# weidafeng/Efficient-SlowFast

Hardware: AMD Instinct MI355X
Metric: clips/sec (8x8 224^2 SlowFast-R50+CMDA, train step fwd+bwd+allreduce+SGD) (higher is better)
Workload: dtype f32

## Files before the change

### efficient-slowfast_amd/sfhip/__init__.py

```python
import ctypes
import os

import torch

_HERE = os.path.dirname(os.path.abspath(__file__))
_LIB_PATH = os.environ.get("SF_LIB") or os.path.join(_HERE, "libsfhip.so")
_lib = None

ACT_NONE, ACT_RELU, ACT_SIGMOID, ACT_SOFTMAX, ACT_HSIGMOID, ACT_RELU6 = 0, 1, 2, 3, 4, 5


def _act(relu):
    return ACT_RELU6 if relu == 6 else (ACT_RELU if relu else ACT_NONE)
SF_EINVAL, SF_EALIGN, SF_ELAUNCH, SF_ENOTTAKEN = -1, -2, -3, -4
_ERR = {-1: "SF_EINVAL (inconsistent descriptor)", -2: "SF_EALIGN", -3: "SF_ELAUNCH (hip launch failed)",
        -4: "SF_ENOTTAKEN (shape not served by this specialised entry point)"}


class SfhipError(RuntimeError):
    pass


class ConvDesc(ctypes.Structure):
    _fields_ = [(n, ctypes.c_int) for n in (
        "N", "Ti", "Hi", "Wi", "Cin", "in_cs", "in_coff", "To", "Ho", "Wo", "Cout", "out_cs", "out_coff",
        "out_cmul", "kT", "kH", "kW", "sT", "sH", "sW", "pT", "pH", "pW", "dT", "dH", "dW", "cin_pad", "act",
        "res_cs", "res_coff", "transposed", "os_T", "os_H", "os_W", "oo_T", "oo_H", "oo_W", "ob_T", "ob_H", "ob_W")]


class PoolDesc(ctypes.Structure):
    _fields_ = [(n, ctypes.c_int) for n in (
        "N", "Ti", "Hi", "Wi", "C", "in_cs", "in_coff", "To", "Ho", "Wo", "out_cs", "out_coff",
        "kT", "kH", "kW", "sT", "sH", "sW", "pT", "pH", "pW", "is_avg")]


EXPORTS = [
    "sf_abi_version", "sf_build_arch", "sf_ncthw_to_ndhwc", "sf_ndhwc_to_ncthw", "sf_conv_fwd", "sf_dwconv_fwd",
    "sf_pool_fwd", "sf_maxpool_fwd_arg", "sf_maxpool_bwd_arg", "sf_tmax_mean_ws_floats", "sf_tmax_mean", "sf_gate_apply", "sf_attn_fwd", "sf_head_act_mean",
    "sf_copy_channels", "sf_channel_stats_ws_floats", "sf_channel_stats", "sf_affine_fwd", "sf_bn_train_stats",
    "sf_conv_wgrad_splits", "sf_conv_wgrad", "sf_bn_bwd_ws_floats", "sf_bn_bwd_reduce", "sf_bn_bwd_apply",
    "sf_attn_bwd", "sf_maxpool_bwd", "sf_tmax_dot", "sf_eca_bwd_apply", "sf_eca_gate_bwd", "sf_bcast_add", "sf_rowdot", "sf_axpy", "sf_act_bwd",
    "sf_dwconv_dgrad", "sf_dwconv_wgrad_ws_floats", "sf_dwconv_wgrad", "sf_gather_add",
    "sf_bn_train_stats_split", "sf_affine_fwd_split", "sf_bn_bwd_reduce_split", "sf_bn_bwd_apply_split",
    "sf_clip_prologue", "sf_conv_wgrad_finish", "sf_bn_bwd_reduce_acc", "sf_row_softmax_fwd", "sf_row_softmax_bwd",
    "sf_attn_bwd_fused_ws_floats", "sf_attn_bwd_fused", "sf_pack_conv_weight", "sf_conv_fwd_ws_floats",
    "sf_conv_fwd_ws", "sf_attn_fwd_ws_floats", "sf_attn_fwd_ws", "sf_affine_fwd_mask", "sf_bn_bwd_apply_first", "sf_maxpool_bwd_first",
    "sf_conv_tune", "sf_conv_stats_ws_floats", "sf_conv_fwd_stats", "sf_bn_train_stats_merge",
    "sf_attn_products_per_fp32", "sf_pack_conv_weights", "sf_attn_bwd_variant", "sf_attn_tune",
    "sf_bx_planes_elems", "sf_bx_split", "sf_bx_split_batched", "sf_conv_rows_parts", "sf_conv_pw_ws_floats", "sf_conv_pw_stats_floats", "sf_conv_fwd_pw", "sf_conv_bx_ws_floats", "sf_conv_fwd_bx", "sf_conv_wgrad_bx_splits",
    "sf_conv_wgrad_bx_ws_floats", "sf_conv_wgrad_bx",
    "sf_conv_fwd_grouped", "sf_conv_wgrad_grouped_splits", "sf_conv_wgrad_grouped", "sf_channel_shuffle",
    "sf_dwconv_wgrad_param", "sf_roi_tpool_fwd", "sf_roi_align_max_fwd", "sf_roi_align_max_bwd", "sf_sigmoid_bwd",
]
_LONG_RET = ("sf_tmax_mean_ws_floats", "sf_channel_stats_ws_floats", "sf_bn_bwd_ws_floats",
             "sf_dwconv_wgrad_ws_floats", "sf_attn_bwd_fused_ws_floats", "sf_conv_fwd_ws_floats",
             "sf_attn_fwd_ws_floats", "sf_conv_stats_ws_floats", "sf_bx_planes_elems", "sf_conv_bx_ws_floats",
             "sf_conv_wgrad_bx_ws_floats")


def lib_path():
    return _LIB_PATH


def lib():
    global _lib
    if _lib is None:
        if not os.path.exists(_LIB_PATH):
            raise SfhipError(
                "libsfhip.so not found at %s — build it with `make -C efficient-slowfast_amd/csrc` "
                "(there is no CPU fallback for the SlowFast hot path)" % _LIB_PATH)
        L = ctypes.CDLL(_LIB_PATH)
        vp, ci, cl = ctypes.c_void_p, ctypes.c_int, ctypes.c_long
        L.sf_abi_version.restype = ci
        L.sf_build_arch.restype = ctypes.c_char_p
        L.sf_ncthw_to_ndhwc.argtypes = [vp, vp] + [ci] * 9 + [vp]
        L.sf_ndhwc_to_ncthw.argtypes = [vp, ci, ci, vp] + [ci] * 5 + [vp]
        L.sf_conv_fwd.argtypes = [ctypes.POINTER(ConvDesc)] + [vp] * 7
        L.sf_dwconv_fwd.argtypes = [ctypes.POINTER(ConvDesc)] + [vp] * 7
        L.sf_pool_fwd.argtypes = [ctypes.POINTER(PoolDesc), vp, vp, vp]
        L.sf_maxpool_fwd_arg.argtypes = [ctypes.POINTER(PoolDesc), vp, vp, vp, vp]
        L.sf_maxpool_bwd_arg.argtypes = [ctypes.POINTER(PoolDesc), vp, vp, ci, ci, vp, ci, ci, ci, vp]
        L.sf_tmax_mean_ws_floats.argtypes = [ci, ci]
        L.sf_tmax_mean_ws_floats.restype = cl
        L.sf_tmax_mean.argtypes = [vp, ci, ci] + [ci] * 6 + [vp, vp, vp]
        L.sf_gate_apply.argtypes = [vp, ci, ci] + [ci] * 6 + [vp, vp, vp, vp, ci, vp, ci, ci, vp]
# ... 54 lines not shown
        L.sf_conv_tune.argtypes = [ci, ci]
        L.sf_attn_tune.argtypes = [ci, ci]
        L.sf_bx_planes_elems.argtypes = [cl, ci]
        L.sf_bx_planes_elems.restype = cl
        L.sf_bx_split.argtypes = [vp, ci, ci, cl, ci, vp, vp]
        L.sf_bx_split_batched.argtypes = [vp, vp, ci, ci, vp]
        L.sf_conv_pw_ws_floats.argtypes = [ctypes.POINTER(ConvDesc), ci]
        L.sf_conv_pw_ws_floats.restype = cl
        L.sf_conv_rows_parts.argtypes = [ctypes.POINTER(ConvDesc)]
        L.sf_conv_pw_stats_floats.argtypes = [ctypes.POINTER(ConvDesc)]
        L.sf_conv_pw_stats_floats.restype = cl
        L.sf_conv_fwd_pw.argtypes = [ctypes.POINTER(ConvDesc)] + [vp] * 9 + [ctypes.POINTER(ctypes.c_int), vp]
        L.sf_conv_bx_ws_floats.argtypes = [ctypes.POINTER(ConvDesc), ci, ci]
        L.sf_conv_bx_ws_floats.restype = cl
        L.sf_conv_fwd_bx.argtypes = [ctypes.POINTER(ConvDesc)] + [vp] * 10
        L.sf_conv_wgrad_bx_splits.argtypes = [ctypes.POINTER(ConvDesc)]
        L.sf_conv_wgrad_bx_ws_floats.argtypes = [ctypes.POINTER(ConvDesc), ci, ci]
        L.sf_conv_wgrad_bx_ws_floats.restype = cl
        L.sf_conv_wgrad_bx.argtypes = [ctypes.POINTER(ConvDesc), vp, vp, vp, ci, ci, vp, vp, vp, vp]
        L.sf_attn_bwd_variant.argtypes = [ci, ci, ci]
        L.sf_row_softmax_fwd.argtypes = [vp, ci, ci, cl, ci, cf, vp]
        L.sf_row_softmax_bwd.argtypes = [vp, ci, ci, vp, ci, ci, cl, ci, cf, vp]
        L.sf_conv_wgrad_finish.argtypes = [vp, ci, ci, ci, ci, ci, ci, vp, ci, vp]
        L.sf_bn_bwd_reduce_acc.argtypes = [vp, ci, ci, vp, ci, ci, vp, ci, ci] + [ci] * 7 + [vp] * 5 + [vp, vp, vp]
        L.sf_bn_train_stats_split.argtypes = [vp, ci, ci, ci, cl, ci, ci, vp, vp, cf, cf] + [vp] * 9
        L.sf_affine_fwd_split.argtypes = [vp, ci, ci] + [ci] * 6 + [vp, vp, vp, ci, ci, ci, ci, vp, ci, ci, ci, vp]
        L.sf_bn_bwd_reduce_split.argtypes = [vp, ci, ci, vp, ci, ci, vp, ci, ci] + [ci] * 8 + [vp] * 5 + [vp]
        L.sf_bn_bwd_apply_split.argtypes = ([vp, ci, ci, vp, ci, ci, vp, ci, ci] + [ci] * 8 + [vp] * 5 +
                                            [vp, ci, ci, vp, ci, ci, vp])
        L.sf_roi_tpool_fwd.argtypes = [vp, ci, ci] + [ci] * 5 + [vp, vp]
        L.sf_roi_align_max_fwd.argtypes = [vp] + [ci] * 4 + [vp, ci, ci, cf, ci, vp, ci, ci, vp, vp]
        L.sf_roi_align_max_bwd.argtypes = [vp, ci, ci, vp, vp] + [ci] * 7 + [cf, ci, vp, ci, ci, ci, vp]
        L.sf_sigmoid_bwd.argtypes = [vp, vp, vp, cl, ci, vp]
        for name in EXPORTS:
            fn = getattr(L, name)
            if name != "sf_build_arch" and name not in _LONG_RET:
                fn.restype = ci
        _lib = L
    return _lib


def _check(rc, what):
    if rc != 0:
        raise SfhipError("%s failed: %s" % (what, _ERR.get(rc, rc)))


CALLS = 0


def _stream():
    global CALLS
    CALLS += 1
    return ctypes.c_void_p(torch.cuda.current_stream().cuda_stream)


def _ptr(t):
    return ctypes.c_void_p(t.data_ptr()) if t is not None else None


EVENT_TRACE = None


def _traced(tag, fn):
    if EVENT_TRACE is None:
        return fn()
    e0 = torch.cuda.Event(enable_timing=True)
# ... 600 lines not shown
    d = ConvDesc(x.N, x.T, x.H, x.W, cin, x.cs, x.coff, dz.T, dz.H, dz.W, cout, 0, 0, 1,
                 kT, kH, kW, stride[0], stride[1], stride[2], padding[0], padding[1], padding[2],
                 dilation[0], dilation[1], dilation[2], cin_pad, ACT_NONE, 0, 0, 0)
    nws = lib().sf_conv_wgrad_bx_ws_floats(ctypes.byref(d), 1 if x_planes is not None else 0,
                                           1 if dz_planes is not None else 0) if cin_pad == cin else 0
    if nws > 0:
        S = lib().sf_conv_wgrad_bx_splits(ctypes.byref(d))
        part = torch.empty((S, cout, kT * kH * kW, cin_pad), dtype=torch.float32, device=x.buf.device)
        ws = torch.empty((nws,), dtype=torch.float32, device=x.buf.device)
        rc = _traced(("conv", dz.rows, kT * kH * kW * cin, cout), lambda: lib().sf_conv_wgrad_bx(
            ctypes.byref(d), x.ptr(), _ptr(x_planes), dz.ptr(), dz.cs, dz.coff, _ptr(dz_planes), _ptr(part), _ptr(ws),
            _stream()))
        if rc in (SF_EALIGN, SF_ENOTTAKEN):
            nws = 0
        else:
            _check(rc, "sf_conv_wgrad_bx")
    if nws <= 0:
        S = lib().sf_conv_wgrad_splits(ctypes.byref(d))
        part = torch.empty((S, cout, kT * kH * kW, cin_pad), dtype=torch.float32, device=x.buf.device)
        _check(_traced(("conv", dz.rows, kT * kH * kW * cin, cout), lambda: lib().sf_conv_wgrad(
            ctypes.byref(d), x.ptr(), dz.ptr(), dz.cs, dz.coff, _ptr(part), _stream())), "sf_conv_wgrad")
    if finish_into is not None:
        dst, real_cin, fold_kw = finish_into
        assert dst.is_contiguous() and dst.dtype == torch.float32
        if S > 128 and cout * kT * kH * kW * cin_pad > 65536:
            part, S = part.sum(0, keepdim=True), 1
        assert dst.numel() == cout * real_cin * kT * kH * kW * max(fold_kw, 1), (dst.shape, cout, real_cin, kernel)
        _check(lib().sf_conv_wgrad_finish(_ptr(part), S, cout, kT * kH * kW, cin_pad, real_cin, fold_kw, _ptr(dst), 1,
                                          _stream()), "sf_conv_wgrad_finish")
        return None
    return part.sum(0) if S > 1 else part[0]


def conv_grouped(x, wp, groups, kernel, stride=(1, 1, 1), padding=(0, 0, 0), dilation=(1, 1, 1), scale=None,
                 bias=None, relu=False, res=None, out=None, shuffle=False, out_reserve=(0, 0)):
    _require_gpu(x.buf, "conv_grouped")
    cout, taps, cin_pad = wp.shape
    kT, kH, kW = kernel
    To = _out_dim(x.T, kT, stride[0], padding[0], dilation[0])
    Ho = _out_dim(x.H, kH, stride[1], padding[1], dilation[1])
    Wo = _out_dim(x.W, kW, stride[2], padding[2], dilation[2])
    if out is None:
        out = new_act(x, x.N, To, Ho, Wo, cout, out_reserve[0], out_reserve[1])
    assert (out.N, out.T, out.H, out.W, out.C) == (x.N, To, Ho, Wo, cout), (out, (x.N, To, Ho, Wo, cout))
    assert x.C % groups == 0 and cout % groups == 0 and cin_pad >= x.C // groups, (x, wp.shape, groups)
    d = ConvDesc(x.N, x.T, x.H, x.W, x.C, x.cs, x.coff, To, Ho, Wo, cout, out.cs, out.coff, 1,
                 kT, kH, kW, stride[0], stride[1], stride[2], padding[0], padding[1], padding[2],
                 dilation[0], dilation[1], dilation[2], cin_pad, _act(relu),
                 res.cs if res is not None else 0, res.coff if res is not None else 0, 0)
    if res is not None:
        assert res.rows == out.rows and res.C == cout
    tag = ("conv", d.N * d.To * d.Ho * d.Wo, taps * (x.C // groups), cout)
    _check(_traced(tag, lambda: lib().sf_conv_fwd_grouped(
        ctypes.byref(d), groups, 1 if shuffle else 0, x.ptr(), _ptr(wp), _ptr(scale), _ptr(bias),
        res.ptr() if res is not None else None, out.ptr(), _stream())), "sf_conv_fwd_grouped")
    return out


def conv_dgrad_grouped(dz, wtp, groups, x_like, kernel, stride=(1, 1, 1), padding=(0, 0, 0), dilation=(1, 1, 1),
                       out=None, accumulate=False):
    _require_gpu(dz.buf, "conv_dgrad_grouped")
    cin, taps, cout_pad = wtp.shape
    if out is None:
        out = new_act(dz, x_like.N, x_like.T, x_like.H, x_like.W, cin)
        accumulate = False
    assert (out.N, out.T, out.H, out.W, out.C) == (x_like.N, x_like.T, x_like.H, x_like.W, cin), (out, x_like)
# ... 10 lines not shown


def conv_wgrad_grouped(x, dz, groups, kernel, stride=(1, 1, 1), padding=(0, 0, 0), dilation=(1, 1, 1),
                       cin_pad=None, finish_into=None):
    _require_gpu(x.buf, "conv_wgrad_grouped")
    cin_g, cout = x.C // groups, dz.C
    assert x.C % groups == 0 and cout % groups == 0
    cin_pad = (cin_g + 15) // 16 * 16 if cin_pad is None else cin_pad
    kT, kH, kW = kernel
    d = ConvDesc(x.N, x.T, x.H, x.W, x.C, x.cs, x.coff, dz.T, dz.H, dz.W, cout, 0, 0, 1,
                 kT, kH, kW, stride[0], stride[1], stride[2], padding[0], padding[1], padding[2],
                 dilation[0], dilation[1], dilation[2], cin_pad, ACT_NONE, 0, 0, 0)
    S = lib().sf_conv_wgrad_grouped_splits(ctypes.byref(d), groups)
    if S <= 0:
        raise SfhipError("sf_conv_wgrad_grouped_splits: %d -> %d channels in %d groups" % (x.C, cout, groups))
    part = torch.empty((S, cout, kT * kH * kW, cin_pad), dtype=torch.float32, device=x.buf.device)
    _check(_traced(("conv", dz.rows, kT * kH * kW * cin_g, cout), lambda: lib().sf_conv_wgrad_grouped(
        ctypes.byref(d), groups, x.ptr(), dz.ptr(), dz.cs, dz.coff, _ptr(part), _stream())), "sf_conv_wgrad_grouped")
    if finish_into is not None:
        dst = finish_into
        assert dst.is_contiguous() and dst.dtype == torch.float32 and dst.numel() == cout * cin_g * kT * kH * kW
        _check(lib().sf_conv_wgrad_finish(_ptr(part), S, cout, kT * kH * kW, cin_pad, cin_g, 0, _ptr(dst), 1,
                                          _stream()), "sf_conv_wgrad_finish")
        return None
    return part.sum(0) if S > 1 else part[0]


def unpack_conv_weight_grad(dwp, shape):
    cout, cin, kT, kH, kW = shape
    return dwp[:, :, :cin].permute(0, 2, 1).reshape(cout, cin, kT, kH, kW).contiguous()


def bn_bwd(dy, y, z, mean, invstd, gamma, relu, rep=1, dres=None, dz_out=None, dgamma_out=None, nsplit=1,
           sync=None, grad_sink=None, mask=None, dres_overwrite=False):
    C = z.C
    dev = z.buf.device
    mean, invstd, gamma = mean.contiguous(), invstd.contiguous(), gamma.detach().contiguous()
    dbeta = torch.empty((nsplit * C,), dtype=torch.float32, device=dev)
    dgamma = torch.empty((nsplit * C,), dtype=torch.float32, device=dev)
    ws = torch.empty((lib().sf_bn_bwd_ws_floats(C),), dtype=torch.float32, device=dev)
    yp, ycs, yco = (y.ptr(), y.cs, y.coff) if y is not None else (None, 0, 0)
    code = 2 if relu == 6 else (1 if relu else 0)
    if mask is not None and relu:
        assert rep == 1 and nsplit == 1 and mask.numel() == z.rows * (C // 4)
        yp, ycs, yco, code = _ptr(mask), C // 4, 0, 3
    head = (dy.ptr(), dy.cs, dy.coff, yp, ycs, yco, z.ptr(), z.cs, z.coff, z.N, z.T, z.H, z.W, C)
    tail = (rep, code, _ptr(mean), _ptr(invstd))
    split = (nsplit,) if nsplit > 1 else ()
    reduce_fn = lib().sf_bn_bwd_reduce_split if nsplit > 1 else lib().sf_bn_bwd_reduce
    apply_fn = lib().sf_bn_bwd_apply_split if nsplit > 1 else lib().sf_bn_bwd_apply
    if dres_overwrite:
        assert dres is not None and nsplit == 1
        apply_fn = lib().sf_bn_bwd_apply_first
    if grad_sink is not None:
        assert nsplit == 1 and dgamma_out is None
        _check(lib().sf_bn_bwd_reduce_acc(*head, *tail, _ptr(dbeta), _ptr(dgamma), _ptr(ws), _ptr(grad_sink[1]),
                                          _ptr(grad_sink[0]), _stream()), "sf_bn_bwd_reduce_acc")
    else:
        _check(reduce_fn(*head, *split, *tail, _ptr(dbeta), _ptr(dgamma), _ptr(ws), _stream()), "sf_bn_bwd_reduce")
    db_apply, dg_apply = (dbeta, dgamma) if sync is None else sync(dbeta, dgamma)
    out = z if dz_out is None else dz_out
    _check(apply_fn(*head, *split, *tail, _ptr(gamma), _ptr(db_apply), _ptr(dg_apply), out.ptr(), out.cs, out.coff,
                    dres.ptr() if dres is not None else None, dres.cs if dres is not None else 0,
                    dres.coff if dres is not None else 0, _stream()), "sf_bn_bwd_apply")
    if dgamma_out is not None:
        if nsplit > 1:
            dgamma_out[0][:C] = dgamma.view(nsplit, C).sum(0)
            dgamma_out[1][:C] = dbeta.view(nsplit, C).sum(0)
        else:
            dgamma_out[0][:C] = dgamma
            dgamma_out[1][:C] = dbeta
    return out, dgamma, dbeta


def maxpool_bwd(x, y, dy, dx, kernel, stride, padding=(0, 0, 0), overwrite=False):
    d = PoolDesc(x.N, x.T, x.H, x.W, x.C, x.cs, x.coff, y.T, y.H, y.W, y.cs, y.coff,
                 kernel[0], kernel[1], kernel[2], stride[0], stride[1], stride[2],
                 padding[0], padding[1], padding[2], 0)
    fn = lib().sf_maxpool_bwd_first if overwrite else lib().sf_maxpool_bwd
    _check(fn(ctypes.byref(d), x.ptr(), y.ptr(), dy.ptr(), dy.cs, dy.coff, dx.ptr(), dx.cs, dx.coff, _stream()),
           "sf_maxpool_bwd")
    return dx


def maxpool_bwd_arg(x_like, arg, dy, dx, kernel, stride, padding=(0, 0, 0), overwrite=False):
    if not (dy.cs % 4 == 0 and dy.coff % 4 == 0 and dx.cs % 4 == 0 and dx.coff % 4 == 0 and
            dy.buf.data_ptr() % 16 == 0 and dx.buf.data_ptr() % 16 == 0):
        return False
    d = PoolDesc(x_like.N, x_like.T, x_like.H, x_like.W, x_like.C, x_like.cs, x_like.coff, dy.T, dy.H, dy.W, dy.cs,
                 dy.coff, kernel[0], kernel[1], kernel[2], stride[0], stride[1], stride[2],
                 padding[0], padding[1], padding[2], 0)
    _check(lib().sf_maxpool_bwd_arg(ctypes.byref(d), _ptr(arg), dy.ptr(), dy.cs, dy.coff, dx.ptr(), dx.cs, dx.coff,
                                    1 if overwrite else 0, _stream()), "sf_maxpool_bwd_arg")
    return True


def tmax_dot(x, alpha, dz):
    out = torch.empty((x.N, x.C), dtype=torch.float32, device=x.buf.device)
    ws = torch.empty((lib().sf_tmax_mean_ws_floats(x.N, x.C),), dtype=torch.float32, device=x.buf.device)
    _check(lib().sf_tmax_dot(x.ptr(), x.cs, x.coff, x.N, x.T, x.H, x.W, x.C, alpha, dz.ptr(), dz.cs, dz.coff,
                             _ptr(out), _ptr(ws), _stream()), "sf_tmax_dot")
    return out


def eca_bwd_apply(x, alpha, dz, gate, dpool, dx):
    _check(lib().sf_eca_bwd_apply(x.ptr(), x.cs, x.coff, x.N, x.T, x.H, x.W, x.C, alpha, dz.ptr(), dz.cs, dz.coff,
                                  _ptr(gate), _ptr(dpool), dx.ptr(), dx.cs, dx.coff, _stream()), "sf_eca_bwd_apply")
# ... 196 lines not shown
```

### efficient-slowfast_amd/slowfast/models/engine.py

```python
import os
import threading
import weakref

import torch
import torch.nn as nn

import sfhip
from sfhip import Act

_tls = threading.local()


class internal(object):

    def __enter__(self):
        self.prev = getattr(_tls, "depth", 0)
        _tls.depth = self.prev + 1

    def __exit__(self, *a):
        _tls.depth = self.prev


def is_internal():
    return getattr(_tls, "depth", 0) > 0
# ... 217 lines not shown

    def __enter__(self):
        self.prev = getattr(_tls, "tape", None)
        _tls.tape = self.t

    def __exit__(self, *a):
        _tls.tape = self.prev


def _colsum(act):
    mean, _ = sfhip.channel_stats(act)
    return mean * float(act.rows)


def _record_conv(x, conv_weight, conv_bias, wp_shape, gsrc, kernel, stride, padding, dilation, x_needs_grad=True,
                 cin=None, unpack=None, fold_kw=0):
    t = tape()
    if t is None:
        return
    cout = conv_weight.shape[0]

    def wgrad(g):
        tgt = t.pgrad_target(conv_weight)
        if tgt is not None:
            real_cin = conv_weight.shape[1]
            sfhip.conv_wgrad(x, g, cout, kernel, stride, padding, dilation, cin=cin, cin_pad=wp_shape[2],
                             finish_into=(tgt, real_cin, fold_kw))
        else:
            dwp = sfhip.conv_wgrad(x, g, cout, kernel, stride, padding, dilation, cin=cin, cin_pad=wp_shape[2])
            t.add_pgrad(conv_weight, unpack(dwp) if unpack else sfhip.unpack_conv_weight_grad(dwp, conv_weight.shape))
        if conv_bias is not None:
            t.add_pgrad(conv_bias, _colsum(g))

    def bwd():
        g = gsrc() if callable(gsrc) else gsrc
        dev = x.buf.device
        if OVERLAP_PATHS and not t.capturing and not t.serial and x_needs_grad and dev.type == "cuda":
            cur = torch.cuda.current_stream(dev)
            wg = _companion_stream(cur)
            _sync_streams(cur, wg)
            with torch.cuda.stream(wg):
                wgrad(g)
            g.buf.record_stream(wg)
            x.buf.record_stream(wg)
            t.joins.add(wg)
        else:
            wgrad(g)
        if x_needs_grad:
            if conv_weight.dim() == 5 and tuple(conv_weight.shape[2:]) == tuple(kernel):
                wtp = _packed_pair(conv_weight)[1]
            else:
                wtp = _cached_t(conv_weight, "_sf_wtp", _key(conv_weight),
                                lambda: sfhip.pack_conv_weight(conv_weight.detach().reshape(
                                    conv_weight.shape[0], conv_weight.shape[1], *kernel).transpose(0, 1).contiguous()))
            fresh = t.grad_of_uninitialised(x)
            if fresh is not None:
                sfhip.conv_dgrad(g, wtp, x, kernel, stride, padding, dilation, out=fresh, accumulate=False)
            else:
                sfhip.conv_dgrad(g, wtp, x, kernel, stride, padding, dilation, out=t.grad_of(x), accumulate=True)

    t.record(bwd)


_PCACHE = {}


_CAPTURE_KEEP = {}


def _keep_if_capturing(obj):
    if getattr(_tls, "capturing", False):
        _CAPTURE_KEEP[id(obj)] = obj
    return obj


def _cached_t(tensor, slot, key, make):
    store = tensor.__dict__.setdefault("_sf_cache", {})
    c = store.get(slot)
    if c is None or c[0] != key:
        with torch.no_grad():
            c = (key, make())
        store[slot] = c
    return _keep_if_capturing(c[1])


_PARAM_EPOCH = 0

# ... 108 lines not shown
    if track:
        bn.__dict__.pop("_sf_affine", None)
        _bump(bn.num_batches_tracked)
    return mean, invstd, scale, shift, 1, bn.weight, None


def bn_train_apply(bn, z, res=None, relu=False, rep=1, out=None, out_reserve=(0, 0), keep=None, out_cmul=1,
                   conv_stats=None):
    check_bn(bn)
    with torch.no_grad():
        mean, invstd, scale, shift, nsplit, gamma_b, sync = _bn_train_stats(bn, z, conv_stats)
    zz = z if keep is None else z.slice(0, keep)
    nk = z.C if keep is None else keep
    if keep is not None:
        assert nsplit == 1, "channel-sliced BN (GhostModule) is only defined for plain BatchNorm3d"
        scale, shift = scale[:keep].contiguous(), shift[:keep].contiguous()
    t = tape()
    shuffled = t is not None and out_cmul != 1
    mk = {} if (t is not None and relu) else None
    if shuffled:
        y = sfhip.affine(zz, scale.contiguous(), shift.contiguous(), res=res, relu=relu, rep=rep, nsplit=nsplit,
                         mask=mk)
    else:
        y = sfhip.affine(zz, scale.contiguous(), shift.contiguous(), res=res, relu=relu, rep=rep, out=out,
                         out_reserve=out_reserve, out_cmul=out_cmul, nsplit=nsplit, mask=mk)
    mask = mk.get("bytes") if mk else None
    if t is not None:
        if _GRAD_SINK:
            dg = db = None
        else:
            dg = torch.zeros(z.C, dtype=torch.float32, device=z.buf.device)
            db = torch.zeros(z.C, dtype=torch.float32, device=z.buf.device)
        sel = slice(None) if nsplit > 1 else slice(0, nk)

        def bwd():
            dres, first = None, False
            if res is not None:
                fresh = t.grad_of_uninitialised(res) if (nsplit == 1 and res.C == zz.C and rep == 1) else None
                dres, first = (fresh, True) if fresh is not None else (t.grad_of(res), False)
            wt = t.pgrad_target(bn.weight) if (nsplit == 1 and getattr(bn, "weight", None) is not None) else None
            bt = t.pgrad_target(bn.bias) if wt is not None else None
            if wt is not None and bt is not None:
                sfhip.bn_bwd(t.grad_of(y), y, zz, mean[sel], invstd[sel], gamma_b[sel], relu, rep=rep, dres=dres,
                             dz_out=zz, sync=sync, grad_sink=(wt, bt), mask=mask, dres_overwrite=first)
            else:
                dg_ = dg if dg is not None else torch.zeros(z.C, dtype=torch.float32, device=z.buf.device)
                db_ = db if db is not None else torch.zeros(z.C, dtype=torch.float32, device=z.buf.device)
                sfhip.bn_bwd(t.grad_of(y), y, zz, mean[sel], invstd[sel], gamma_b[sel], relu, rep=rep, dres=dres,
                             dz_out=zz, dgamma_out=(dg_, db_), nsplit=nsplit, sync=sync, mask=mask,
                             dres_overwrite=first)
            if keep is not None and keep < z.C:
                rest = z.slice(keep, z.C - keep)
                sfhip.axpy(rest, rest, alpha=0.0, accumulate=False)
            if (wt is None or bt is None) and getattr(bn, "weight", None) is not None:
                t.add_pgrad(bn.weight, dg_)
                t.add_pgrad(bn.bias, db_)

        t.record(bwd)
    if shuffled:
        return copy_channels(y, out, out_cmul=out_cmul)
    return y


def bn_affine(bn, conv_bias=None):
    check_bn(bn)
    stat = bn.bn if _sub_bn(bn) else bn
    w = getattr(bn, "weight", None)
    b = getattr(bn, "bias", None)

    def make():
        inv = 1.0 / torch.sqrt(stat.running_var + stat.eps)
        scale = w * inv if w is not None else inv
        bias = -stat.running_mean * scale
        if b is not None:
            bias = bias + b
        if conv_bias is not None:
            bias = bias + scale * conv_bias
        return scale.detach().contiguous(), bias.detach().contiguous()

    return _cached(bn, "_sf_affine", _key(w, b, stat.running_mean, stat.running_var, conv_bias), make)

# ... 466 lines not shown
```

### include/sfhip.h

```cpp
#ifndef SFHIP_H
#define SFHIP_H
#ifdef __cplusplus
extern "C" {
#endif

#define SF_OK 0
#define SF_EINVAL (-1)
#define SF_EALIGN (-2)
#define SF_ELAUNCH (-3)
#define SF_ENOTTAKEN (-4)

#define SF_ACT_NONE 0
#define SF_ACT_RELU 1
#define SF_ACT_SIGMOID 2
#define SF_ACT_SOFTMAX 3
#define SF_ACT_HSIGMOID 4
#define SF_ACT_RELU6 5

int sf_abi_version(void);
const char* sf_build_arch(void);

int sf_ncthw_to_ndhwc(const float* src, float* dst, int N, int C, int T, int H, int W,
                      int cpad, int ph, int pw, int Wp, void* stream);
int sf_ndhwc_to_ncthw(const float* src, int cs, int coff, float* dst, int N, int C, int T, int H,
// ... 91 lines not shown
long sf_channel_stats_ws_floats(int C);
int sf_channel_stats(const float* x, int cs, int coff, long rows, int C, float* mean, float* var, float* ws,
                     void* stream);
int sf_bn_train_stats(const float* x, int cs, int coff, long rows, int C, const float* gamma, const float* beta,
                      float eps, float momentum, float* run_mean, float* run_var, float* mean, float* var,
                      float* invstd, float* scale, float* shift, float* ws, void* stream);
int sf_bn_train_stats_merge(const float* parts_ws, int parts, int C, const float* gamma, const float* beta, float eps,
                            float momentum, float* run_mean, float* run_var, float* mean, float* var, float* invstd,
                            float* scale, float* shift, void* stream);
int sf_affine_fwd(const float* x, int cs, int coff, int N, int T, int H, int W, int C, const float* scale,
                  const float* bias, const float* res, int res_cs, int res_coff, int act, int rep, float* out,
                  int out_cs, int out_coff, int out_cmul, void* stream);

int sf_head_act_mean(const float* logits, int B, int P, int K, int act, float* out, void* stream);

int sf_copy_channels(const float* in, int in_cs, int in_coff, float* out, int out_cs, int out_coff,
                     int out_cmul, long rows, int C, void* stream);
int sf_channel_shuffle(const float* in, int in_cs, int in_coff, float* out, int out_cs, int out_coff, int groups,
                       long rows, int C, int accumulate, void* stream);

int sf_conv_wgrad_splits(const sf_conv_desc* d);
int sf_conv_wgrad_bx_splits(const sf_conv_desc* d);
long sf_conv_wgrad_bx_ws_floats(const sf_conv_desc* d, int have_x_planes, int have_dz_planes);
int sf_conv_wgrad_bx(const sf_conv_desc* d, const float* x, const unsigned short* x_planes, const float* dz, int dz_cs,
                     int dz_coff, const unsigned short* dz_planes, float* partial, float* ws, void* stream);
int sf_conv_wgrad(const sf_conv_desc* d, const float* x, const float* dz, int dz_cs, int dz_coff,
                  float* partial, void* stream);
int sf_conv_wgrad_grouped_splits(const sf_conv_desc* d, int groups);
int sf_conv_wgrad_grouped(const sf_conv_desc* d, int groups, const float* x, const float* dz, int dz_cs, int dz_coff,
                          float* partial, void* stream);
int sf_conv_wgrad_finish(const float* partial, int S, int Cout, int packed_taps, int cin_pad, int Cin, int fold_kw,
                         float* dst, int accumulate, void* stream);

#define SF_BN_MASK_BYTES 3
long sf_bn_bwd_ws_floats(int C);
int sf_affine_fwd_mask(const float* x, int cs, int coff, int N, int T, int H, int W, int C, const float* scale,
                       const float* bias, const float* res, int res_cs, int res_coff, int act, float* out,
                       int out_cs, int out_coff, unsigned char* mask, void* stream);
int sf_bn_bwd_reduce(const float* dy, int dy_cs, int dy_coff, const float* y, int y_cs, int y_coff,
                     const float* z, int z_cs, int z_coff, int N, int T, int H, int W, int C, int rep, int relu,
                     const float* mean, const float* invstd, float* dbeta, float* dgamma, float* ws, void* stream);
int sf_bn_bwd_reduce_acc(const float* dy, int dy_cs, int dy_coff, const float* y, int y_cs, int y_coff,
                         const float* z, int z_cs, int z_coff, int N, int T, int H, int W, int C, int rep, int relu,
                         const float* mean, const float* invstd, float* dbeta, float* dgamma, float* ws,
                         float* dbeta_acc, float* dgamma_acc, void* stream);
int sf_bn_bwd_apply(const float* dy, int dy_cs, int dy_coff, const float* y, int y_cs, int y_coff,
                    const float* z, int z_cs, int z_coff, int N, int T, int H, int W, int C, int rep, int relu,
                    const float* mean, const float* invstd, const float* gamma, const float* dbeta,
                    const float* dgamma, float* dz, int dz_cs, int dz_coff, float* dres, int dres_cs,
                    int dres_coff, void* stream);
int sf_bn_bwd_apply_first(const float* dy, int dy_cs, int dy_coff, const float* y, int y_cs, int y_coff,
                          const float* z, int z_cs, int z_coff, int N, int T, int H, int W, int C, int rep, int relu,
                          const float* mean, const float* invstd, const float* gamma, const float* dbeta,
                          const float* dgamma, float* dz, int dz_cs, int dz_coff, float* dres, int dres_cs,
                          int dres_coff, void* stream);

int sf_maxpool_bwd(const sf_pool_desc* d, const float* x, const float* y, const float* dy, int dy_cs,
                   int dy_coff, float* dx, int dx_cs, int dx_coff, void* stream);
int sf_maxpool_bwd_first(const sf_pool_desc* d, const float* x, const float* y, const float* dy, int dy_cs,
                         int dy_coff, float* dx, int dx_cs, int dx_coff, void* stream);

int sf_tmax_dot(const float* x, int cs, int coff, int N, int T, int H, int W, int C, int alpha, const float* dz,
                int dz_cs, int dz_coff, float* out, float* ws, void* stream);
int sf_eca_bwd_apply(const float* x, int cs, int coff, int N, int T, int H, int W, int C, int alpha,
                     const float* dz, int dz_cs, int dz_coff, const float* gate, const float* dpool, float* dx,
                     int dx_cs, int dx_coff, void* stream);

int sf_eca_gate_bwd(const float* dg, const float* pooled, const float* w3, int N, int C, float dpool_scale,
                    float* gate, float* dpool, float* dw3, void* stream);

int sf_dwconv_dgrad(const sf_conv_desc* d, const float* dz, int dz_cs, int dz_coff, const float* w_packed,
                    float* dx, int dx_cs, int dx_coff, int C, void* stream);
long sf_dwconv_wgrad_ws_floats(const sf_conv_desc* d, int C);
int sf_dwconv_wgrad(const sf_conv_desc* d, const float* x, const float* dz, int dz_cs, int dz_coff, int C,
                    float* dw, float* ws, void* stream);
int sf_dwconv_wgrad_param(const sf_conv_desc* d, const float* x, const float* dz, int dz_cs, int dz_coff, int C,
                          float* dw_param, int accumulate, float* ws, void* stream);
int sf_gather_add(const float* in, int in_cs, int in_coff, int in_cmul, float* out, int out_cs, int out_coff,
                  long rows, int C, int accumulate, void* stream);

int sf_bcast_add(float* g, int cs, int coff, int N, long rows_per_n, int C, const float* v, float scale,
                 void* stream);
int sf_rowdot(const float* a, int a_cs, int a_coff, const float* b, int b_cs, int b_coff, long rows, int C,
              float scale, float* out, void* stream);
int sf_axpy(const float* a, int a_cs, int a_coff, float alpha, float* out, int out_cs, int out_coff, long rows,
            int C, int accumulate, void* stream);
int sf_bn_train_stats_split(const float* x, int cs, int coff, int N, long rows_per_sample, int C, int nsplit,
                            const float* gamma, const float* beta, float eps, float momentum, float* run_mean,
// ... 39 lines not shown
```

Baseline: 150.6.

## Bundle conv and BN backward launches into single native entry points with cached plans

Adds native sf_conv_bwd and sf_bn_bwd entry points that issue dgrad, wgrad, the finish step and the BN reduce/apply kernels from one host call. The conv path records an event, runs dgrad on the main stream and wgrad on a companion stream, and caches per-shape descriptor plans on the weight. BN backward pre-slices mean, invstd and gamma once in the forward pass. The goal is to cut Python/ctypes dispatch and per-call descriptor building in the backward pass, at the cost of more code paths and a pooled-event scheme that could reuse events across streams.

```diff
diff --git a/efficient-slowfast_amd/csrc/bwd_bundle.hip b/efficient-slowfast_amd/csrc/bwd_bundle.hip
--- /dev/null
+++ b/efficient-slowfast_amd/csrc/bwd_bundle.hip
@@ -0,0 +1,158 @@
+#include "common.h"
+#include <mutex>
+
+namespace {
+
+constexpr int EV_DEVICES = 16;
+constexpr int EV_PER_DEVICE = 8;
+
+struct EventPool {
+  std::mutex mu;
+  hipEvent_t ev[EV_DEVICES][EV_PER_DEVICE] = {};
+  bool made[EV_DEVICES] = {};
+  unsigned next[EV_DEVICES] = {};
+
+  hipEvent_t take() {
+    int dev = 0;
+    if (hipGetDevice(&dev) != hipSuccess || dev < 0 || dev >= EV_DEVICES) return nullptr;
+    std::lock_guard<std::mutex> lock(mu);
+    if (!made[dev]) {
+      for (int i = 0; i < EV_PER_DEVICE; ++i)
+        if (hipEventCreateWithFlags(&ev[dev][i], hipEventDisableTiming) != hipSuccess) {
+          for (int j = 0; j < i; ++j) (void)hipEventDestroy(ev[dev][j]);
+          return nullptr;
+        }
+      made[dev] = true;
+    }
+    return ev[dev][next[dev]++ % EV_PER_DEVICE];
+  }
+
+  ~EventPool() {
+    for (int d = 0; d < EV_DEVICES; ++d)
+      if (made[d])
+        for (int i = 0; i < EV_PER_DEVICE; ++i) (void)hipEventDestroy(ev[d][i]);
+  }
+};
+
+EventPool g_events;
+
+inline bool refused(int rc) { return rc == SF_EALIGN || rc == SF_ENOTTAKEN; }
+inline long lmax(long a, long b) { return a > b ? a : b; }
+
+long dgrad_ws_need(const sf_conv_desc* d, bool planes, bool split_k) {
+  if (!split_k) return 0;
+  long n = sf_conv_fwd_ws_floats(d);
+  if (planes) n = lmax(n, lmax(sf_conv_pw_ws_floats(d, 1), sf_conv_bx_ws_floats(d, 0, 1)));
+  return lmax(n, 0);
+}
+
+int dgrad_launch(const sf_conv_desc* d, const float* dz, const float* w, const unsigned short* planes,
+                 const float* res, float* dx, float* ws, bool split_k, void* stream) {
+  if (split_k && planes) {
+    if (sf_conv_pw_ws_floats(d, 1) > 0) {
+      const int rc = sf_conv_fwd_pw(d, dz, w, planes, nullptr, nullptr, res, dx, ws, nullptr, nullptr, stream);
+      if (!refused(rc)) return rc;
+    }
+    if (sf_conv_bx_ws_floats(d, 0, 1) > 0) {
+      const int rc = sf_conv_fwd_bx(d, dz, nullptr, w, planes, nullptr, nullptr, res, dx, ws, stream);
+      if (!refused(rc)) return rc;
+    }
+  }
+  if (split_k && sf_conv_fwd_ws_floats(d) > 0)
+    return sf_conv_fwd_ws(d, dz, w, nullptr, nullptr, res, dx, ws, stream);
+  return sf_conv_fwd(d, dz, w, nullptr, nullptr, res, dx, stream);
+}
+
+}
+
+extern "C" int sf_conv_bwd(int n_dgrad, const sf_conv_desc* dd, const float* const* dw,
+                           const unsigned short* const* dw_planes, const float* dz, const float* dres, float* dx,
+                           float* dws, long dws_floats, const sf_conv_desc* wd, const float* x, int dz_cs, int dz_coff,
+                           float* part, long part_floats, float* wws, long wws_floats, float* finish_dst,
+                           int finish_cin, int fold_kw, int* splits, int split_k, void* stream, void* companion) {
+  if (n_dgrad < 0 || (n_dgrad > 0 && (!dd || !dw || !dw_planes || !dx)) || !dz) return SF_EINVAL;
+  if (wd && (!x || !part || part_floats <= 0)) return SF_EINVAL;
+  if (!wd && n_dgrad == 0) return SF_EINVAL;
+  for (int i = 0; i < n_dgrad; ++i) {
+    if (!dw[i]) return SF_EINVAL;
+    const long need = dgrad_ws_need(&dd[i], dw_planes[i] != nullptr, split_k != 0);
+    if (need > dws_floats || (need > 0 && !dws)) return SF_EINVAL;
+  }
+  long bx_ws = 0;
+  int S_bx = 0, S_f32 = 0;
+  long per_split = 0;
+  if (wd) {
+    per_split = (long)wd->Cout * wd->kT * wd->kH * wd->kW * wd->cin_pad;
+    if (per_split <= 0) return SF_EINVAL;
+    if (wd->cin_pad == wd->Cin) bx_ws = sf_conv_wgrad_bx_ws_floats(wd, 0, 0);
+    if (bx_ws > 0) {
+      S_bx = sf_conv_wgrad_bx_splits(wd);
+      if (S_bx <= 0 || bx_ws > wws_floats || !wws) return SF_EINVAL;
+    }
+    S_f32 = sf_conv_wgrad_splits(wd);
+    if (S_f32 <= 0) return SF_EINVAL;
+    if (lmax(S_bx, S_f32) * per_split > part_floats) return SF_EINVAL;
+  }
+  void* wstream = stream;
+  if (wd && companion && companion != stream) {
+    hipEvent_t ev = g_events.take();
+    if (!ev) return SF_ELAUNCH;
+    if (hipEventRecord(ev, (hipStream_t)stream) != hipSuccess) return SF_ELAUNCH;
+    for (int i = 0; i < n_dgrad; ++i) {
+      const int rc = dgrad_launch(&dd[i], dz, dw[i], dw_planes[i], dres, dx, dws, split_k != 0, stream);
+      if (rc != SF_OK) return rc;
+    }
+    if (hipStreamWaitEvent((hipStream_t)companion, ev, 0) != hipSuccess) return SF_ELAUNCH;
+    wstream = companion;
+  }
+  int S = 0;
+  if (wd) {
+    int rc = SF_ENOTTAKEN;
+    if (bx_ws > 0) {
+      rc = sf_conv_wgrad_bx(wd, x, nullptr, dz, dz_cs, dz_coff, nullptr, part, wws, wstream);
+      S = S_bx;
+    }
+    if (refused(rc)) {
+      rc = sf_conv_wgrad(wd, x, dz, dz_cs, dz_coff, part, wstream);
+      S = S_f32;
+    }
+    if (rc != SF_OK) return rc;
+    if (finish_dst) {
+      rc = sf_conv_wgrad_finish(part, S, wd->Cout, wd->kT * wd->kH * wd->kW, wd->cin_pad, finish_cin, fold_kw,
+                                finish_dst, 1, wstream);
+      if (rc != SF_OK) return rc;
+    }
+  }
+  if (splits) *splits = S;
+  if (wstream == stream)
+    for (int i = 0; i < n_dgrad; ++i) {
+      const int rc = dgrad_launch(&dd[i], dz, dw[i], dw_planes[i], dres, dx, dws, split_k != 0, stream);
+      if (rc != SF_OK) return rc;
+    }
+  return SF_OK;
+}
+
+extern "C" int sf_bn_bwd(const float* dy, int dy_cs, int dy_coff, const float* y, int y_cs, int y_coff, const float* z,
+                         int z_cs, int z_coff, int N, int T, int H, int W, int C, int rep, int relu, const float* mean,
+                         const float* invstd, const float* gamma, float* dbeta, float* dgamma, float* ws,
+                         float* dbeta_acc, float* dgamma_acc, float* dz, int dz_cs, int dz_coff, float* dres,
+                         int dres_cs, int dres_coff, int dres_first, void* stream) {
+  if (!gamma || !dz || (dres_first && !dres)) return SF_EINVAL;
+  if (relu == SF_BN_MASK_BYTES &&
+      ((dz_cs % 4) != 0 || (dz_coff % 4) != 0 || !sf_aligned16(dz) ||
+       (dres && ((dres_cs % 4) != 0 || (dres_coff % 4) != 0 || !sf_aligned16(dres)))))
+    return SF_EINVAL;
+  int rc;
+  if (dbeta_acc || dgamma_acc)
+    rc = sf_bn_bwd_reduce_acc(dy, dy_cs, dy_coff, y, y_cs, y_coff, z, z_cs, z_coff, N, T, H, W, C, rep, relu, mean,
+                              invstd, dbeta, dgamma, ws, dbeta_acc, dgamma_acc, stream);
+  else
+    rc = sf_bn_bwd_reduce(dy, dy_cs, dy_coff, y, y_cs, y_coff, z, z_cs, z_coff, N, T, H, W, C, rep, relu, mean, invstd,
+                          dbeta, dgamma, ws, stream);
+  if (rc != SF_OK) return rc;
+  if (dres_first)
+    return sf_bn_bwd_apply_first(dy, dy_cs, dy_coff, y, y_cs, y_coff, z, z_cs, z_coff, N, T, H, W, C, rep, relu, mean,
+                                 invstd, gamma, dbeta, dgamma, dz, dz_cs, dz_coff, dres, dres_cs, dres_coff, stream);
+  return sf_bn_bwd_apply(dy, dy_cs, dy_coff, y, y_cs, y_coff, z, z_cs, z_coff, N, T, H, W, C, rep, relu, mean, invstd,
+                         gamma, dbeta, dgamma, dz, dz_cs, dz_coff, dres, dres_cs, dres_coff, stream);
+}
diff --git a/efficient-slowfast_amd/sfhip/__init__.py b/efficient-slowfast_amd/sfhip/__init__.py
--- a/efficient-slowfast_amd/sfhip/__init__.py
+++ b/efficient-slowfast_amd/sfhip/__init__.py
@@ -51,6 +51,7 @@
     "sf_conv_wgrad_bx_ws_floats", "sf_conv_wgrad_bx",
     "sf_conv_fwd_grouped", "sf_conv_wgrad_grouped_splits", "sf_conv_wgrad_grouped", "sf_channel_shuffle",
     "sf_dwconv_wgrad_param", "sf_roi_tpool_fwd", "sf_roi_align_max_fwd", "sf_roi_align_max_bwd", "sf_sigmoid_bwd",
+    "sf_conv_bwd", "sf_bn_bwd",
 ]
 _LONG_RET = ("sf_tmax_mean_ws_floats", "sf_channel_stats_ws_floats", "sf_bn_bwd_ws_floats",
              "sf_dwconv_wgrad_ws_floats", "sf_attn_bwd_fused_ws_floats", "sf_conv_fwd_ws_floats",
@@ -171,6 +172,10 @@
         L.sf_roi_align_max_fwd.argtypes = [vp] + [ci] * 4 + [vp, ci, ci, cf, ci, vp, ci, ci, vp, vp]
         L.sf_roi_align_max_bwd.argtypes = [vp, ci, ci, vp, vp] + [ci] * 7 + [cf, ci, vp, ci, ci, ci, vp]
         L.sf_sigmoid_bwd.argtypes = [vp, vp, vp, cl, ci, vp]
+        L.sf_conv_bwd.argtypes = [ci, vp, vp, vp, vp, vp, vp, vp, cl, ctypes.POINTER(ConvDesc), vp, ci, ci, vp, cl, vp, cl,
+                                  vp, ci, ci, ctypes.POINTER(ctypes.c_int), ci, vp, vp]
+        L.sf_bn_bwd.argtypes = ([vp, ci, ci, vp, ci, ci, vp, ci, ci] + [ci] * 7 + [vp] * 8 + [vp, ci, ci, vp, ci, ci, ci,
+                                                                                             vp])
         for name in EXPORTS:
             fn = getattr(L, name)
             if name != "sf_build_arch" and name not in _LONG_RET:
@@ -837,6 +842,156 @@
     return part.sum(0) if S > 1 else part[0]
 
 
+class _ConvBwdPlan(object):
+    __slots__ = ("n", "descs", "classes", "want_planes", "wptrs", "pptrs", "dws", "wd", "part", "wws", "wtotal",
+                 "zero_first", "add", "big_finish", "splits")
+
+
+def _dgrad_desc(dz, out, cin, cout_pad, kernel, stride, padding, dilation, accumulate):
+    return ConvDesc(dz.N, dz.T, dz.H, dz.W, dz.C, dz.cs, dz.coff, out.T, out.H, out.W, cin, out.cs, out.coff, 1,
+                    kernel[0], kernel[1], kernel[2], stride[0], stride[1], stride[2], padding[0], padding[1],
+                    padding[2], dilation[0], dilation[1], dilation[2], cout_pad, ACT_NONE,
+                    out.cs if accumulate else 0, out.coff if accumulate else 0, 1)
+
+
+def _conv_bwd_plan(x, dz, wt_shape, cout, kernel, stride, padding, dilation, cin, cin_pad, out, accumulate):
+    L = lib()
+    p = _ConvBwdPlan()
+    descs, classes = [], []
+    p.zero_first, p.add = False, accumulate
+    if out is not None:
+        dcin, _, cout_pad = wt_shape
+        if max(stride) > 1 and tuple(dilation) == (1, 1, 1) and (accumulate or (out.coff == 0 and out.cs == out.C)):
+            every = all(_residue_taps(k, s, pd, a)[1] and (full - a + s - 1) // s > 0
+                        for k, s, pd, full in zip(kernel, stride, padding, (out.T, out.H, out.W)) for a in range(s))
+            p.add = accumulate or not every
+            p.zero_first = not accumulate and not every
+            for at in range(stride[0]):
+                ot, tt = _residue_taps(kernel[0], stride[0], padding[0], at)
+                for ah in range(stride[1]):
+                    oh, th = _residue_taps(kernel[1], stride[1], padding[1], ah)
+                    for aw in range(stride[2]):
+                        ow, tw = _residue_taps(kernel[2], stride[2], padding[2], aw)
+                        dims = [(full - a + s - 1) // s
+                                for full, a, s in zip((out.T, out.H, out.W), (at, ah, aw), stride)]
+                        if not (tt and th and tw) or min(dims) <= 0:
+                            continue
+                        classes.append((at, ah, aw, tuple(kernel), tuple(stride), tuple(padding)))
+                        descs.append(ConvDesc(
+                            dz.N, dz.T, dz.H, dz.W, dz.C, dz.cs, dz.coff, dims[0], dims[1], dims[2], dcin, out.cs,
+                            out.coff, 1, len(tt), len(th), len(tw), 1, 1, 1, -ot[0], -oh[0], -ow[0], 1, 1, 1, cout_pad,
+                            ACT_NONE, out.cs, out.coff, 0, stride[0], stride[1], stride[2], at, ah, aw, out.T, out.H,
+                            out.W))
+        else:
+            classes.append(None)
+            descs.append(_dgrad_desc(dz, out, dcin, cout_pad, kernel, stride, padding, dilation, accumulate))
+    p.n = len(descs)
+    p.descs = (ConvDesc * max(p.n, 1))(*descs)
+    p.classes = classes
+    p.want_planes, p.dws = [], 0
+    for d in descs:
+        n_pw = n_bx = 0
+        if SPLIT_K and wt_shape[2] == d.Cin:
+            n_pw = L.sf_conv_pw_ws_floats(ctypes.byref(d), 1)
+            n_bx = L.sf_conv_bx_ws_floats(ctypes.byref(d), 0, 1)
+        p.want_planes.append(n_pw > 0 or n_bx > 0)
+        p.dws = max(p.dws, n_pw, n_bx, L.sf_conv_fwd_ws_floats(ctypes.byref(d)) if SPLIT_K else 0)
+    p.wptrs = (ctypes.c_void_p * max(p.n, 1))()
+    p.pptrs = (ctypes.c_void_p * max(p.n, 1))()
+    kT, kH, kW = kernel
+    p.wd = ConvDesc(x.N, x.T, x.H, x.W, cin, x.cs, x.coff, dz.T, dz.H, dz.W, cout, 0, 0, 1,
+                    kT, kH, kW, stride[0], stride[1], stride[2], padding[0], padding[1], padding[2],
+                    dilation[0], dilation[1], dilation[2], cin_pad, ACT_NONE, 0, 0, 0)
+    p.wws = L.sf_conv_wgrad_bx_ws_floats(ctypes.byref(p.wd), 0, 0) if cin_pad == cin else 0
+    S = max(L.sf_conv_wgrad_bx_splits(ctypes.byref(p.wd)) if p.wws > 0 else 0, L.sf_conv_wgrad_splits(ctypes.byref(p.wd)))
+    p.wws = max(p.wws, 0)
+    per = cout * kT * kH * kW * cin_pad
+    p.part = (S * per + 127) // 128 * 128
+    p.wtotal = p.part + p.wws
+    p.big_finish = S > 128 and per > 65536
+    p.splits = ctypes.c_int(0)
+    return p
+
+
+def conv_bwd(x, dz, wt_packed, cout, kernel, stride=(1, 1, 1), padding=(0, 0, 0), dilation=(1, 1, 1), cin=None,
+             cin_pad=None, finish_into=None, out=None, accumulate=False, companion=None, plans=None):
+    _require_gpu(x.buf, "conv_bwd")
+    cin = x.C if cin is None else cin
+    cin_pad = (cin + 15) // 16 * 16 if cin_pad is None else cin_pad
+    dev = x.buf.device
+    if wt_packed is not None and out is None:
+        out = new_act(dz, x.N, x.T, x.H, x.W, wt_packed.shape[0])
+        accumulate = False
+    if out is not None:
+        assert (out.N, out.T, out.H, out.W, out.C) == (x.N, x.T, x.H, x.W, wt_packed.shape[0]), (out, x)
+    key = (x.buf.shape, x.coff, x.C, dz.buf.shape, dz.coff, dz.C, kernel, stride, padding, dilation, cin, cin_pad,
+           None if out is None else (out.cs, out.coff, wt_packed.shape), accumulate, SPLIT_K)
+    plan = plans.get(key) if plans is not None else None
+    for attempt in (0, 1):
+        if plan is None:
+            plan = _conv_bwd_plan(x, dz, wt_packed.shape if out is not None else None, cout, tuple(kernel),
+                                  tuple(stride), tuple(padding), tuple(dilation), cin, cin_pad, out, accumulate)
+            if plans is not None:
+                plans[key] = plan
+        if plan.big_finish and finish_into is not None:
+            with torch.cuda.stream(companion if companion is not None else torch.cuda.current_stream()):
+                conv_wgrad(x, dz, cout, kernel, stride, padding, dilation, cin=cin, cin_pad=cin_pad,
+                           finish_into=finish_into)
+            if out is not None:
+                conv_dgrad(dz, wt_packed, x, kernel, stride, padding, dilation, out=out, accumulate=accumulate)
+            return out, None
+        if plan.zero_first:
+            out.buf.zero_()
+        for i, cls in enumerate(plan.classes):
+            w = wt_packed
+            if cls is not None:
+                store = wt_packed.__dict__.setdefault("_sf_classes", {})
+                w = store.get(cls)
+                if w is None:
+                    w = _class_weights(wt_packed, store, cls[3], cls[4], cls[5])[cls]
+            plan.wptrs[i] = w.data_ptr()
+            plan.pptrs[i] = _weight_planes(w).data_ptr() if plan.want_planes[i] else None
+        dws = torch.empty((plan.dws,), dtype=torch.float32, device=dev) if plan.dws > 0 else None
+        global CALLS
+        CALLS += 1
+        cur = torch.cuda.current_stream()
+        raw = None
+        if finish_into is not None:
+            dst, real_cin, fold_kw = finish_into
+            assert dst.is_contiguous() and dst.dtype == torch.float32
+            assert dst.numel() == cout * real_cin * kernel[0] * kernel[1] * kernel[2] * max(fold_kw, 1), (dst.shape, cout)
+            raw = torch.cuda.caching_allocator_alloc(plan.wtotal * 4, dev, companion if companion is not None else cur)
+            part_ptr = raw
+        else:
+            dst, real_cin, fold_kw = None, 0, 0
+            with torch.cuda.stream(companion if companion is not None else cur):
+                wbuf = torch.empty((plan.wtotal,), dtype=torch.float32, device=dev)
+            part_ptr = wbuf.data_ptr()
+        try:
+            rc = lib().sf_conv_bwd(
+                plan.n, plan.descs, plan.wptrs, plan.pptrs, dz.ptr(), out.ptr() if (out is not None and plan.add) else None,
+                out.ptr() if out is not None else None, _ptr(dws), plan.dws, ctypes.byref(plan.wd), x.ptr(), dz.cs,
+                dz.coff, part_ptr, plan.part, (part_ptr + plan.part * 4) if plan.wws > 0 else None, plan.wws,
+                _ptr(dst), real_cin, fold_kw, ctypes.byref(plan.splits), 1 if SPLIT_K else 0, cur.cuda_stream,
+                companion.cuda_stream if companion is not None else None)
+        finally:
+            if raw is not None:
+                torch.cuda.caching_allocator_delete(raw)
+        if rc == SF_EINVAL and attempt == 0 and plans is not None:
+            plan = None
+            continue
+        _check(rc, "sf_conv_bwd")
+        break
+    if finish_into is not None:
+        return out, None
+    S = plan.splits.value
+    per = cout * kernel[0] * kernel[1] * kernel[2] * cin_pad
+    with torch.cuda.stream(companion if companion is not None else cur):
+        part = wbuf[:S * per].view(S, cout, kernel[0] * kernel[1] * kernel[2], cin_pad)
+        dwp = part.sum(0) if S > 1 else part[0]
+    return out, dwp
+
+
 def conv_grouped(x, wp, groups, kernel, stride=(1, 1, 1), padding=(0, 0, 0), dilation=(1, 1, 1), scale=None,
                  bias=None, relu=False, res=None, out=None, shuffle=False, out_reserve=(0, 0)):
     _require_gpu(x.buf, "conv_grouped")
@@ -913,10 +1068,13 @@
 
 
 def bn_bwd(dy, y, z, mean, invstd, gamma, relu, rep=1, dres=None, dz_out=None, dgamma_out=None, nsplit=1,
-           sync=None, grad_sink=None, mask=None, dres_overwrite=False):
+           sync=None, grad_sink=None, mask=None, dres_overwrite=False, bundled=True):
     C = z.C
     dev = z.buf.device
     mean, invstd, gamma = mean.contiguous(), invstd.contiguous(), gamma.detach().contiguous()
+    if bundled and nsplit == 1 and sync is None:
+        return _bn_bwd_bundled(dy, y, z, mean, invstd, gamma, relu, rep, dres, dz_out, dgamma_out, grad_sink, mask,
+                               dres_overwrite)
     dbeta = torch.empty((nsplit * C,), dtype=torch.float32, device=dev)
     dgamma = torch.empty((nsplit * C,), dtype=torch.float32, device=dev)
     ws = torch.empty((lib().sf_bn_bwd_ws_floats(C),), dtype=torch.float32, device=dev)
@@ -954,6 +1112,42 @@
     return out, dgamma, dbeta
 
 
+_BN_WS_FLOATS = {}
+
+
+def _bn_bwd_bundled(dy, y, z, mean, invstd, gamma, relu, rep, dres, dz_out, dgamma_out, grad_sink, mask, first):
+    C = z.C
+    nws = _BN_WS_FLOATS.get(C)
+    if nws is None:
+        nws = _BN_WS_FLOATS[C] = lib().sf_bn_bwd_ws_floats(C)
+    cp = (C + 3) // 4 * 4
+    buf = torch.empty((2 * cp + nws,), dtype=torch.float32, device=z.buf.device)
+    base = buf.data_ptr()
+    yp, ycs, yco = (y.ptr(), y.cs, y.coff) if y is not None else (None, 0, 0)
+    code = 2 if relu == 6 else (1 if relu else 0)
+    if mask is not None and relu:
+        assert rep == 1 and mask.numel() == z.rows * (C // 4)
+        yp, ycs, yco, code = mask.data_ptr(), C // 4, 0, 3
+    if first:
+        assert dres is not None
+    if grad_sink is not None:
+        assert dgamma_out is None
+    out = z if dz_out is None else dz_out
+    zb, ob = z.buf, out.buf
+    _check(lib().sf_bn_bwd(
+        dy.buf.data_ptr(), dy.cs, dy.coff, yp, ycs, yco, zb.data_ptr(), z.cs, z.coff, zb.shape[0], zb.shape[1],
+        zb.shape[2], zb.shape[3], C, rep, code, mean.data_ptr(), invstd.data_ptr(), gamma.data_ptr(), base,
+        base + 4 * cp, base + 8 * cp, grad_sink[1].data_ptr() if grad_sink is not None else None,
+        grad_sink[0].data_ptr() if grad_sink is not None else None, ob.data_ptr(), out.cs, out.coff,
+        dres.buf.data_ptr() if dres is not None else None, dres.cs if dres is not None else 0,
+        dres.coff if dres is not None else 0, 1 if first else 0, _stream()), "sf_bn_bwd")
+    dbeta, dgamma = buf[:C], buf[cp:cp + C]
+    if dgamma_out is not None:
+        dgamma_out[0][:C] = dgamma
+        dgamma_out[1][:C] = dbeta
+    return out, dgamma, dbeta
+
+
 def maxpool_bwd(x, y, dy, dx, kernel, stride, padding=(0, 0, 0), overwrite=False):
     d = PoolDesc(x.N, x.T, x.H, x.W, x.C, x.cs, x.coff, y.T, y.H, y.W, y.cs, y.coff,
                  kernel[0], kernel[1], kernel[2], stride[0], stride[1], stride[2],
diff --git a/efficient-slowfast_amd/slowfast/models/engine.py b/efficient-slowfast_amd/slowfast/models/engine.py
--- a/efficient-slowfast_amd/slowfast/models/engine.py
+++ b/efficient-slowfast_amd/slowfast/models/engine.py
@@ -273,9 +273,43 @@
         if conv_bias is not None:
             t.add_pgrad(conv_bias, _colsum(g))
 
+    kernel, stride, padding, dilation = tuple(kernel), tuple(stride), tuple(padding), tuple(dilation)
+    paired = conv_weight.dim() == 5 and tuple(conv_weight.shape[2:]) == kernel
+    real_cin = conv_weight.shape[1]
+    on_gpu = x.buf.device.type == "cuda"
+    plans = conv_weight.__dict__.setdefault("_sf_bwd_plans", {})
+
+    def dgrad_weight():
+        if paired:
+            return _packed_pair(conv_weight)[1]
+        return _cached_t(conv_weight, "_sf_wtp", _key(conv_weight),
+                         lambda: sfhip.pack_conv_weight(conv_weight.detach().reshape(
+                             conv_weight.shape[0], conv_weight.shape[1], *kernel).transpose(0, 1).contiguous()))
+
+    def bwd_bundled(g, tgt):
+        wg = None
+        if OVERLAP_PATHS and not t.capturing and not t.serial and x_needs_grad:
+            wg = _companion_stream(torch.cuda.current_stream(x.buf.device))
+        out, acc = None, False
+        if x_needs_grad:
+            out = t.grad_of_uninitialised(x)
+            if out is None:
+                out, acc = t.grad_of(x), True
+        sfhip.conv_bwd(x, g, dgrad_weight() if x_needs_grad else None, cout, kernel, stride, padding, dilation,
+                       cin=cin, cin_pad=wp_shape[2], finish_into=(tgt, real_cin, fold_kw), out=out, accumulate=acc,
+                       companion=wg, plans=plans)
+        if wg is not None:
+            g.buf.record_stream(wg)
+            x.buf.record_stream(wg)
+            t.joins.add(wg)
+
     def bwd():
         g = gsrc() if callable(gsrc) else gsrc
         dev = x.buf.device
+        if on_gpu and conv_bias is None and sfhip.EVENT_TRACE is None:
+            tgt = t.pgrad_target(conv_weight)
+            if tgt is not None:
+                return bwd_bundled(g, tgt)
         if OVERLAP_PATHS and not t.capturing and not t.serial and x_needs_grad and dev.type == "cuda":
             cur = torch.cuda.current_stream(dev)
             wg = _companion_stream(cur)
@@ -288,12 +322,7 @@
         else:
             wgrad(g)
         if x_needs_grad:
-            if conv_weight.dim() == 5 and tuple(conv_weight.shape[2:]) == tuple(kernel):
-                wtp = _packed_pair(conv_weight)[1]
-            else:
-                wtp = _cached_t(conv_weight, "_sf_wtp", _key(conv_weight),
-                                lambda: sfhip.pack_conv_weight(conv_weight.detach().reshape(
-                                    conv_weight.shape[0], conv_weight.shape[1], *kernel).transpose(0, 1).contiguous()))
+            wtp = dgrad_weight()
             fresh = t.grad_of_uninitialised(x)
             if fresh is not None:
                 sfhip.conv_dgrad(g, wtp, x, kernel, stride, padding, dilation, out=fresh, accumulate=False)
@@ -468,6 +497,8 @@
             dg = torch.zeros(z.C, dtype=torch.float32, device=z.buf.device)
             db = torch.zeros(z.C, dtype=torch.float32, device=z.buf.device)
         sel = slice(None) if nsplit > 1 else slice(0, nk)
+        with torch.no_grad():
+            mean_s, invstd_s, gamma_s = mean[sel].contiguous(), invstd[sel].contiguous(), gamma_b.detach()[sel].contiguous()
 
         def bwd():
             dres, first = None, False
@@ -477,12 +508,12 @@
             wt = t.pgrad_target(bn.weight) if (nsplit == 1 and getattr(bn, "weight", None) is not None) else None
             bt = t.pgrad_target(bn.bias) if wt is not None else None
             if wt is not None and bt is not None:
-                sfhip.bn_bwd(t.grad_of(y), y, zz, mean[sel], invstd[sel], gamma_b[sel], relu, rep=rep, dres=dres,
+                sfhip.bn_bwd(t.grad_of(y), y, zz, mean_s, invstd_s, gamma_s, relu, rep=rep, dres=dres,
                              dz_out=zz, sync=sync, grad_sink=(wt, bt), mask=mask, dres_overwrite=first)
             else:
                 dg_ = dg if dg is not None else torch.zeros(z.C, dtype=torch.float32, device=z.buf.device)
                 db_ = db if db is not None else torch.zeros(z.C, dtype=torch.float32, device=z.buf.device)
-                sfhip.bn_bwd(t.grad_of(y), y, zz, mean[sel], invstd[sel], gamma_b[sel], relu, rep=rep, dres=dres,
+                sfhip.bn_bwd(t.grad_of(y), y, zz, mean_s, invstd_s, gamma_s, relu, rep=rep, dres=dres,
                              dz_out=zz, dgamma_out=(dg_, db_), nsplit=nsplit, sync=sync, mask=mask,
                              dres_overwrite=first)
             if keep is not None and keep < z.C:
diff --git a/include/sfhip.h b/include/sfhip.h
--- a/include/sfhip.h
+++ b/include/sfhip.h
@@ -147,6 +147,12 @@
 int sf_conv_wgrad_finish(const float* partial, int S, int Cout, int packed_taps, int cin_pad, int Cin, int fold_kw,
                          float* dst, int accumulate, void* stream);
 
+int sf_conv_bwd(int n_dgrad, const sf_conv_desc* dd, const float* const* dw, const unsigned short* const* dw_planes,
+                const float* dz, const float* dres, float* dx, float* dws, long dws_floats, const sf_conv_desc* wd,
+                const float* x, int dz_cs, int dz_coff, float* part, long part_floats, float* wws, long wws_floats,
+                float* finish_dst, int finish_cin, int fold_kw, int* splits, int split_k, void* stream,
+                void* companion);
+
 #define SF_BN_MASK_BYTES 3
 long sf_bn_bwd_ws_floats(int C);
 int sf_affine_fwd_mask(const float* x, int cs, int coff, int N, int T, int H, int W, int C, const float* scale,
@@ -169,6 +175,12 @@
                           const float* mean, const float* invstd, const float* gamma, const float* dbeta,
                           const float* dgamma, float* dz, int dz_cs, int dz_coff, float* dres, int dres_cs,
                           int dres_coff, void* stream);
+
+int sf_bn_bwd(const float* dy, int dy_cs, int dy_coff, const float* y, int y_cs, int y_coff, const float* z, int z_cs,
+              int z_coff, int N, int T, int H, int W, int C, int rep, int relu, const float* mean, const float* invstd,
+              const float* gamma, float* dbeta, float* dgamma, float* ws, float* dbeta_acc, float* dgamma_acc,
+              float* dz, int dz_cs, int dz_coff, float* dres, int dres_cs, int dres_coff, int dres_first,
+              void* stream);
 
 int sf_maxpool_bwd(const sf_pool_desc* d, const float* x, const float* y, const float* dy, int dy_cs,
                    int dy_coff, float* dx, int dx_cs, int dx_coff, void* stream);
```

Result: no change. 150.4 (-0.1%).
